# bcgsc/abyss

Measured on AMD Instinct MI355X. Metric: Mk-mers/s inserted+extended (abyss-bloom-dbg, k=64); unitig bit-exact, higher is better.
Workload: dtype u64

## Files before the change

abyss_amd/csrc/abg_core.h:

```cpp
#pragma once

#include <stdint.h>
#include <stddef.h>

#if defined(__HIPCC__)
#include <hip/hip_runtime.h>
#define ABG_HD __host__ __device__ __forceinline__
#define ABG_HDN __host__ __device__
#define ABG_HDX __host__ __device__ __attribute__((noinline))
#else
#define ABG_HD inline
#define ABG_HDN
#define ABG_HDX
#endif

namespace abg {

constexpr int MAX_NW = 6;
constexpr int MAX_HASHES = 32;
constexpr unsigned FP_TRIM = 5;

enum Dir : int { FORWARD = 0, REVERSE = 1 };
enum Sense : int { SENSE = 0, ANTISENSE = 1 };

// ... 1106 lines not shown
	uint32_t o = *counter; *counter = o + 1; return o;
}
#endif

#if defined(__HIP_DEVICE_COMPILE__)
ABG_HD void wave_count_add(uint64_t* counter, bool want)
{
	const uint64_t m = __ballot(want ? 1 : 0);
	if (m && (int)__lane_id() == __ffsll((unsigned long long)m) - 1) atomicAdd((unsigned long long*)counter, (unsigned long long)__popcll(m));
}
#else
ABG_HD void wave_count_add(uint64_t* counter, bool want) { if (want) *counter += 1; }
#endif

#if defined(__HIP_DEVICE_COMPILE__)
ABG_HD uint32_t wave_rank(bool want, uint32_t& count)
{
	const uint64_t m = __ballot(want ? 1 : 0);
	count = (uint32_t)__popcll(m);
	return (uint32_t)__popcll(m & ((1ull << __lane_id()) - 1));
}
#else
ABG_HD uint32_t wave_rank(bool want, uint32_t& count) { count = want ? 1u : 0u; return 0; }
#endif

#if defined(__HIP_DEVICE_COMPILE__)
ABG_HD uint64_t wu_cas_u64(uint64_t* p, uint64_t expect, uint64_t val, bool coop)
{
	if (!coop) return cas_u64(p, expect, val);
	uint64_t r = 0;
	if (__lane_id() == 0) r = cas_u64(p, expect, val);
	return ((uint64_t)(uint32_t)__builtin_amdgcn_readfirstlane((int)(r >> 32)) << 32) |
	       (uint32_t)__builtin_amdgcn_readfirstlane((int)(uint32_t)r);
}
ABG_HD uint32_t wu_atomic_min_u32(uint32_t* p, uint32_t v, bool coop)
{
	if (!coop) return atomic_min_u32(p, v);
	uint32_t r = 0;
	if (__lane_id() == 0) r = atomic_min_u32(p, v);
	return (uint32_t)__builtin_amdgcn_readfirstlane((int)r);
}
ABG_HD uint32_t wu_atomic_add_u32(uint32_t* p, uint32_t v, bool coop)
{
	if (!coop) return atomic_add_u32(p, v);
	uint32_t r = 0;
	if (__lane_id() == 0) r = atomic_add_u32(p, v);
// ... 1001 lines not shown
```

abyss_amd/csrc/abg_engine.h:

```cpp
#pragma once
#include "abg_walk.h"

#include <algorithm>
#include <chrono>
#include <cstdio>
#include <cstdlib>
#include <cstring>
#include <functional>
#include <future>
#include <string>
#include <type_traits>
#include <vector>

namespace abg {

struct Failure { int code; std::string msg; };
constexpr int FAIL_INVAL = -1, FAIL_NOMEM = -3, FAIL_INTERNAL = -4;
[[noreturn]] inline void fail_now(int code, const std::string& msg) { throw Failure{ code, msg }; }
inline std::string strf(const char* fmt, unsigned long long a = 0, unsigned long long b = 0)
{
	char buf[256];
	snprintf(buf, sizeof buf, fmt, a, b);
	return buf;
}
// ... 31 lines not shown
	uint32_t p2_crowded = 1u << 18;
	uint32_t p2_starved_growth = 2;
	uint32_t p2_starved = 6144;
	uint32_t slice_filter = 0;
	bool solid_plane = true;
	uint32_t classify_slots = 65536;
	uint32_t cls_both_max_mb = 1024;
	bool cls_both = true;
	bool prefetch_classify = true;
	uint32_t memo_log2 = 0;
	bool memo = true;
	uint32_t p2_max_candidates = 1u << 18;
	uint32_t t_tags = 1024;
	uint32_t commit_incremental = 1;
	uint32_t commit_dirty_max = 4096;
	uint32_t commit_dirty_log2 = 26;
	uint32_t guide_stride = 4;
	uint32_t guide_log2_max = 31;
	bool guide_seen = true;
	bool link_duplicates = true;
	bool par_commit = true;
	bool overlap_bins = true;
	bool overlap_purity = true;
	uint32_t dist_hash_all_ranks = 2;
	uint32_t dist_route_min_ranks = 4;
	uint64_t keep_insert_scratch_bytes = 16ull << 30;
	uint64_t par_commit_max_bytes = 16ull << 30;
	int verbose = 0;
};

struct Counters {
	uint64_t solid_reads = 0, visited_reads = 0, reads_processed = 0, bases_assembled = 0,
	         contig_id = 0;
};

struct BaseCodes {
	uint8_t t[256];
	BaseCodes()
	{
		for (int i = 0; i < 256; i++) t[i] = 0xFF;
		t['A'] = t['a'] = 0; t['C'] = t['c'] = 1; t['G'] = t['g'] = 2; t['T'] = t['t'] = 3;
	}
};
template <class T>
struct NoInitAlloc : std::allocator<T> {
	template <class U> struct rebind { using other = NoInitAlloc<U>; };
// ... 412 lines not shown
constexpr uint32_t TILE_PAIRS_MEAN = 1u << ABG_TILE_PAIRS_LOG2;
constexpr uint32_t TILE_SORT_MAX = 3u * TILE_PAIRS_MEAN / 2;
struct TilePair { uint32_t hlo, hhi, tj; };
constexpr uint32_t TP_T_BITS = 28, TP_T_MASK = (1u << TP_T_BITS) - 1;
ABG_HD uint64_t tp_h(const TilePair& r) { return ((uint64_t)r.hhi << 32) | r.hlo; }
ABG_HD uint32_t tp_t(const TilePair& r) { return r.tj & TP_T_MASK; }
ABG_HD uint32_t tp_j(const TilePair& r) { return r.tj >> TP_T_BITS; }
constexpr uint32_t LEAD_BIT = 0x80000000u;
struct TileEnv {
	Params p; uint8_t* cnt;
	uint64_t lo, m;
	const uint64_t* h0;
	TilePair* bins; uint32_t cap;
	uint32_t* tcur;
	uint32_t* lead;
	uint8_t* opflag;
	uint8_t* tgt;
	uint8_t* pendf;
	uint32_t* flags;
	uint32_t benign = 1;
	uint32_t lead_js = 2;
	uint32_t count_max = 0x7FFFFFFFu;
	const uint8_t* cval = nullptr;
	uint32_t* bad = nullptr;
	uint32_t bad_mask = 0;
	uint8_t* wmask = nullptr;
	uint32_t* chg = nullptr;
	uint32_t* colist = nullptr;
	uint8_t* cocnt = nullptr;
	uint32_t glog2 = 0;
};
constexpr uint32_t CO_MAX_PASSES = 15;
constexpr uint8_t PEND_NO = 0, PEND_ROUNDS = 1, PEND_CANDIDATE = 2;
constexpr uint32_t CO_LANE_SHIFT = 26, CO_MORE = 1u << 25, CO_SLOT_MASK = CO_MORE - 1, CO_DEAD = 0xFFFFFFFFu;
template <class Get, class Put>
ABG_HD void kmer_hash_run(const Params& p, Get get, uint32_t j0, uint32_t j1, Put put)
{
	if (j0 >= j1) return;
	const unsigned k = p.k;
	if (p.mask) {
		const MaskTab& m = *p.mask;
		uint64_t fh = 0, rh = 0, df = 0, dr = 0;
		for (unsigned i = 0; i < k; i++) {
			fh = srol1(fh) ^ seed_of(get(j0 + i));
			rh = srol1(rh) ^ seed_of(3u - get(j0 + k - 1 - i));
		}
// ... 257 lines not shown
		atomic_min_u64(&first[s], ((uint64_t)tp_t(r) << TILE_IDX_BITS) | i);
		atomic_add_u32(&info[s], 1);
	});
	sy.barrier();
	if (keep) {
		TilePair fst[TILE_PURITY_PER];
#pragma unroll
		for (uint32_t q = 0; q < TILE_PURITY_PER; q++) {
			const uint32_t i = tid + q * nt;
			fst[q] = bin[i < n ? (uint32_t)(first[slot[q] & 0xFFFFu] & ((1u << TILE_IDX_BITS) - 1u)) : 0u];
		}
#pragma unroll
		for (uint32_t q = 0; q < TILE_PURITY_PER; q++) {
			const uint32_t i = tid + q * nt;
			const TilePair& r = mine[q]; const TilePair& f = fst[q];
			if (i < n && (r.hlo != f.hlo || r.hhi != f.hhi || ((r.tj ^ f.tj) != 0 && tp_t(r) == tp_t(f)))) atomic_or_u32(&info[slot[q] & 0xFFFFu], 0x80000000u);
		}
	} else
	pairs([&](const TilePair& r, uint32_t, uint32_t s, uint32_t) {
		const TilePair f = bin[(uint32_t)(first[s] & ((1u << TILE_IDX_BITS) - 1u))];
		if (r.hlo != f.hlo || r.hhi != f.hhi || ((r.tj ^ f.tj) != 0 && tp_t(r) == tp_t(f))) atomic_or_u32(&info[s], 0x80000000u);
	});
	sy.barrier();
	pairs([&](const TilePair& r, uint32_t, uint32_t s, uint32_t) {
		const uint32_t inf = info[s], t = tp_t(r);
		if ((inf >> 31) || (inf & 0x7FFFFFFFu) >= e.count_max) {
			const uint32_t bit = e.p.nh <= 8 ? (1u << tp_j(r)) : 0xFFu;
			atomic_or_u32((uint32_t*)e.opflag + (t >> 2), bit << (8 * (t & 3u)));
			return;
		}
		if (tp_j(r) >= e.lead_js) return;
		const bool first_op = (uint32_t)(first[s] >> TILE_IDX_BITS) == t;
		e.lead[t] = (inf & 0x7FFFFFFFu) | (first_op ? LEAD_BIT : 0u);
	});
}
ABG_HD uint32_t bad_slot(const TileEnv& e, uint64_t pos) { return (uint32_t)(pos ^ (pos >> 27)) & e.bad_mask; }
ABG_HD void mark_bad(const TileEnv& e, uint64_t h, unsigned js)
{
	for (unsigned j = 0; j < e.p.nh && j < 8; j++)
		if ((js >> j) & 1u) { const uint32_t s = bad_slot(e, pos_i(e.p, h, j)); atomic_or_u32(&e.bad[s >> 5], 1u << (s & 31u)); }
}
ABG_HD bool any_bad(const TileEnv& e, uint64_t h, unsigned js)
{
	bool b = false;
	for (unsigned j = 0; j < e.p.nh && j < 8; j++)
		if ((js >> j) & 1u) { const uint32_t s = bad_slot(e, pos_i(e.p, h, j)); b |= ((e.bad[s >> 5] >> (s & 31u)) & 1u) != 0; }
	return b;
}
ABG_HD void op_verdict(const TileEnv& e, uint64_t t, uint8_t& tgt, uint8_t& pend, uint32_t& centry)
{
	tgt = 0; pend = PEND_ROUNDS; centry = 0;
	if (e.flags[0]) return;
	const uint32_t fl = e.opflag[t], L = e.lead[t], n = L & ~LEAD_BIT;
	if (fl && (!n || e.p.nh > 8 || !e.benign)) { if (e.bad && e.p.nh <= 8) mark_bad(e, e.h0[t], fl); return; }
	if (!fl && !(L & LEAD_BIT)) { pend = PEND_NO; return; }
	const uint64_t h = e.h0[t];
	unsigned mp = 256, ms = 256;
	unsigned cs[8];
	for (unsigned j0 = 0; j0 < e.p.nh; j0 += 4) {
		unsigned c[4];
#pragma unroll
		for (unsigned q = 0; q < 4; q++) {
			const unsigned jq = j0 + q < e.p.nh ? j0 + q : 0u;
			c[q] = e.cval ? 255u - e.cval[t * e.p.nh + jq] : e.cnt[pos_i(e.p, h, jq)];
		}
#pragma unroll
		for (unsigned q = 0; q < 4; q++) {
			const unsigned j = j0 + q;
			if (j >= e.p.nh) continue;
			if (j < 8) cs[j] = c[q];
			if ((fl >> j) & 1u) ms = c[q] < ms ? c[q] : ms; else mp = c[q] < mp ? c[q] : mp;
		}
	}
	const unsigned tg = mp + n > 255 ? 255u : mp + n;
	if (fl && ms < tg) {
		if (!e.bad) return;
// ... 125 lines not shown
	if (ld_coherent(&e.flags[0])) return;
	const uint64_t nbins = (e.m - e.lo + BIN_COUNTERS - 1) >> BIN_BITS;
	uint32_t nb[TILE_SPLIT], n = 0;
#pragma unroll
	for (uint32_t q = 0; q < TILE_SPLIT; q++) {
		const uint64_t bi = tile * TILE_SPLIT + q;
		const uint32_t f = bi < nbins ? ld_coherent(&e.tcur[bi]) : 0u;
		nb[q] = f < e.cap ? f : e.cap;
		n += nb[q];
	}
	if (!n) return;
	const uint32_t tid = sy.tid(), nt = sy.nthreads();
	const uint64_t base = e.lo + (tile << TILE_BITS);
	const uint32_t span = (uint32_t)(e.m - base < TILE_COUNTERS ? e.m - base : TILE_COUNTERS);
	uint64_t* l8 = (uint64_t*)lds;
	const uint64_t* g8 = (const uint64_t*)(e.cnt + base);
	for (uint32_t i = tid; i < span / 8; i += nt) l8[i] = g8[i];
	sy.barrier();
	bool any = false;
	constexpr uint32_t PER = TILE_SPLIT * ((TILE_SORT_MAX + 1023) / 1024);
	uint32_t mine[PER];
	uint32_t kept = 0;
	const bool keep = e.bad && nt >= 1024;
	auto raise = [&](const TilePair& r, bool first) -> bool {
		const uint8_t tg = e.tgt[tp_t(r)];
		if (!tg) return false;
		const uint32_t off = (uint32_t)(pos_i(e.p, tp_h(r), tp_j(r)) - e.lo) & (TILE_COUNTERS - 1);
		if (first && keep && kept < PER) mine[kept++] = off | ((uint32_t)tg << 16);
		if (lds[off] < tg) { lds[off] = tg; return true; }
		return false;
	};
#pragma unroll
	for (uint32_t q = 0; q < TILE_SPLIT; q++) {
		const TilePair* bin = e.bins + (tile * TILE_SPLIT + q) * e.cap;
		for (uint32_t i = tid; i < nb[q]; i += nt) any |= raise(bin[i], true);
	}
	if (e.bad) {
		for (bool again = any; sy.any(again);) {
			again = false;
			if (keep) {
#pragma unroll
				for (uint32_t q = 0; q < PER; q++)
					if (q < kept) { const uint32_t off = mine[q] & 0xFFFFu; const uint8_t tg = (uint8_t)(mine[q] >> 16); if (lds[off] < tg) { lds[off] = tg; again = true; } }
			} else {
				for (uint32_t q = 0; q < TILE_SPLIT; q++) {
					const TilePair* bin = e.bins + (tile * TILE_SPLIT + q) * e.cap;
					for (uint32_t i = tid; i < nb[q]; i += nt) again |= raise(bin[i], false);
				}
			}
		}
	}
	if (sy.any(any)) {
		uint64_t* o8 = (uint64_t*)(e.cnt + base);
		for (uint32_t i = tid; i < span / 8; i += nt) o8[i] = l8[i];
	}
}
struct SortEnv {
	TileEnv e; uint64_t T, np;
	uint64_t* key; uint32_t* val;
	uint64_t* sid;
	uint32_t* start;
	uint8_t* impure;
};
struct FSortKeys {
	SortEnv s;
	ABG_HD void operator()(uint64_t q, uint32_t) const
	{
		const uint64_t t = q / s.e.p.nh; const unsigned j = (unsigned)(q - t * s.e.p.nh);
		s.key[q] = pos_i(s.e.p, s.e.h0[t], j);
		s.val[q] = (uint32_t)t << 4 | j;
// ... 13 lines not shown
};
struct FSegImpure {
	SortEnv s;
	ABG_HD void operator()(uint64_t i, uint32_t) const
	{
		const uint64_t g = s.sid[i] - 1, f = s.start[g];
		if (i == f) return;
		const uint32_t v = s.val[i], vf = s.val[f];
		if (s.e.h0[v >> 4] != s.e.h0[vf >> 4] || (v >> 4) == (vf >> 4)) s.impure[g] = 1;
	}
};
struct FSegJudge {
	SortEnv s;
	ABG_HD void operator()(uint64_t i, uint32_t) const
	{
		const uint64_t g = s.sid[i] - 1;
		const uint32_t f = s.start[g], cnt = s.start[g + 1] - f, v = s.val[i], t = v >> 4, j = v & 15u;
		if (s.impure[g] || cnt >= s.e.count_max) {
			const uint32_t bit = s.e.p.nh <= 8 ? (1u << j) : 0xFFu;
			atomic_or_u32((uint32_t*)s.e.opflag + (t >> 2), bit << (8 * (t & 3u)));
			return;
		}
		if (j >= s.e.lead_js) return;
		s.e.lead[t] = cnt | ((s.val[f] >> 4) == t ? LEAD_BIT : 0u);
	}
};
struct FSegApply {
	SortEnv s;
	ABG_HD void operator()(uint64_t i, uint32_t) const
	{
		const uint8_t tg = s.e.tgt[s.val[i] >> 4];
		if (!tg) return;
		const uint64_t pos = s.key[i];
		uint32_t* w = (uint32_t*)(s.e.cnt + (pos & ~3ull));
		const unsigned sh = 8u * (unsigned)(pos & 3u);
		for (uint32_t old = *w;;) {
			if (((old >> sh) & 0xFFu) >= tg) return;
			const uint32_t want = (old & ~(0xFFu << sh)) | ((uint32_t)tg << sh);
			const uint32_t got = cas_u32(w, old, want);
			if (got == old) return;
			old = got;
		}
	}
};
struct FClaimList {
	Params p; const uint64_t* h0; const uint32_t* pend; uint64_t* claim; uint64_t cmask; uint32_t epoch;
// ... 1628 lines not shown
			casc_.levels = cfg_.cascade_levels;
			casc_.level_words = (m_ + 31) / 32;
			casc_.bits = (uint32_t*)be_.alloc(casc_.levels * casc_.level_words * 4);
			be_.memset(casc_.bits, 0, casc_.levels * casc_.level_words * 4);
			cnt_ = (uint8_t*)be_.alloc(8);
			vis_bytes_ = 8;
		} else {
			const uint64_t dev = be_.device_mem_bytes();
			cnt_deferred_ = cfg_.slice_filter == 1 || (cfg_.slice_filter == 0 && dev && (double)m_ * 1.3 > (double)dev * 0.9);
			if (!cnt_deferred_) {
				cnt_ = (uint8_t*)be_.alloc(m_ + 64 * (MAX_RANKS + 1));
				be_.memset(cnt_, 0, m_);
			}
			vis_bytes_ = (m_ / 8 + 4 + 3) & ~3ull;
		}
		vis_ = (uint8_t*)be_.alloc(vis_bytes_);
		be_.memset(vis_, 0, vis_bytes_);
		cstate_ = (CommitState*)be_.alloc(sizeof(CommitState));
		be_.memset(cstate_, 0, sizeof(CommitState));
		scal_ = (uint64_t*)be_.alloc(64);
	}
	~Engine()
	{
		free_counters(); be_.free(vis_); if (both_) be_.free(both_); be_.free(cstate_); be_.free(scal_);
		free_archive();
		if (casc_.bits) be_.free(casc_.bits);
		if (mask_d_) be_.free(mask_d_);
		if (T_) be_.free(T_);
		if (Tk_) { be_.free(Tk_); be_.free(Tv_); }
		if (pcA_) be_.free(pcA_);
		if (la_pool_c_) be_.free(la_pool_c_);
		if (la_pool_c2_) be_.free(la_pool_c2_);
		if (guide_tab_) be_.free(guide_tab_);
		if (guide_seen_) be_.free(guide_seen_);
		if (gtab_.hmin) free_tab(gtab_);
		free_shared();
		free_insert();
		free_walk();
		if (cend_.hmin) free_tab(cend_);
		if (memo_tab_.hmin) free_tab(memo_tab_);
		if (plane_) be_.free(plane_);
		if (wstats_) be_.free(wstats_);
	}
	void reset()
	{
		if (casc_.bits) be_.memset(casc_.bits, 0, casc_.levels * casc_.level_words * 4);
// ... 248 lines not shown
	}
	void load_packed(const Batch& b, const uint64_t* koff_h) { load_packed(b, cut_ranges_host(koff_h, b.n)); }
	void load_packed(const Batch& b) { load_packed(b, cut_ranges(b.koff, b.n)); }
	void load_packed(const Batch& b, const std::vector<OpRange>& ranges)
	{
		need_counters();
		cnt_loaded_ = true;
		{
			uint32_t len0 = 0;
			if (b.n) be_.d2h(&len0, b.len, 4);
			const uint32_t nk0 = len0 >= p_.k ? len0 - p_.k + 1 : 0;
			const uint32_t parts = (nk0 + 31) / 32;
			hash_run_ = parts ? std::min<uint32_t>(32, std::max<uint32_t>(8, (nk0 + parts - 1) / parts)) : 8;
		}
		ensure_insert();
		memo_valid_ = false; plane_valid_ = false;
		last_rounds_ = 0;
		const bool pipe = tiled_ && bins_alt_ != nullptr && !routed();
		for (size_t i = 0; i < ranges.size(); i++) {
			if (!pipe) { insert_range(b, ranges[i], false); continue; }
			if (i == 0) stage_bins(b, ranges[0]);
			be_.wait_side_scope();
			std::swap(h0_, h0_alt_); std::swap(bins_, bins_alt_); std::swap(tcur_, tcur_alt_); stage_flag_ ^= 1u;
			if (lead_alt_) { std::swap(lead_, lead_alt_); std::swap(opflag_, opflag_alt_); }
			const bool staged = staged_ok_;
			purity_done_ = staged && staged_purity_;
			const uint32_t cur_flag = stage_flag_ ^ 1u;
			stage_next_ = nullptr;
			if (i + 1 < ranges.size()) stage_next_ = [this, &b, &ranges, i]() { stage_bins(b, ranges[i + 1]); };
			insert_range(b, ranges[i], staged, 2 + cur_flag);
			if (stage_next_) { stage_next_(); stage_next_ = nullptr; }
		}
	}
	void stage_bins(const Batch& b, const OpRange& rg)
	{
		const uint64_t s = rg.s, e = rg.e;
		const uint64_t T = rg.k1 - rg.k0;
		staged_ok_ = false;
		if (T == 0 || T > batch_ops_ || T >= 0xFFFFFFFFull) return;
		Batch v = b;
		v.woff = b.woff + s; v.len = b.len + s; v.n = e - s; v.koff = b.koff + s;
		const uint64_t kbase = rg.k0;
		uint32_t* flag = pend_n_ + 2 + stage_flag_;
		uint64_t* h0 = h0_alt_;
		const bool part = dist();
		TileEnv te{ p_, cnt_, part ? own_lo_ : 0, part ? own_lo_ + own_span_ : m_, h0_alt_, bins_alt_, tile_cap_, tcur_alt_, lead_alt_ ? lead_alt_ : lead_,
			opflag_alt_ ? opflag_alt_ : opflag_, tgt_, pendf_, flag, cfg_.benign_sharers ? 1u : 0u, part ? 16u : 2u, part ? 254u : 0x7FFFFFFFu };
		const uint64_t R = part ? (uint64_t)comm_.world : 1, me = part ? (uint64_t)comm_.rank : 0;
		if (part && R > cfg_.dist_hash_all_ranks) {
			const uint64_t chunk = ((T + R - 1) / R + 7) & ~7ull;
			std::vector<uint64_t> c(R, chunk * 8), d(R);
			for (uint64_t q = 0; q < R; q++) d[q] = q * chunk * 8;
			const uint64_t a = std::min(T, me * chunk), bnd = std::min(T, a + chunk);
			if (bnd > a) {
				be_.side_scope_begin("hash_staged");
				dispatch_nw([&](auto nw) { FHashOps<(decltype(nw)::value & 7)> f{ p_, v, h0, bnd, kbase, a, hash_run_ }; be_.launch((bnd - a + hash_run_ - 1) / hash_run_, f, "hash_ops"); });
				be_.side_scope_end();
				be_.wait_side_scope();
			}
			c_all_gather_v(h0, c.data(), d.data());
		}
		be_.side_scope_begin("hash_bin_staged");
		be_.memset(tcur_alt_, 0, ntiles_ * 4);
		be_.memset(flag, 0, 4);
		be_.memset(ccur_, 0, ncoarse_ * 4);
		if (!part || R <= cfg_.dist_hash_all_ranks)
			dispatch_nw([&](auto nw) { FHashOps<(decltype(nw)::value & 7)> f{ p_, v, h0, T, kbase, 0, hash_run_ }; be_.launch((T + hash_run_ - 1) / hash_run_, f, "hash_ops"); });
		BinEnv bn{ te, T, coarse_, coarse_cap_, ccur_, cshift_, ncoarse_ };
		FBinCoarse f1{ bn };
		be_.launch_tiles((T + BIN_CHUNK_OPS - 1) / BIN_CHUNK_OPS, f1, "bin_coarse");
		const uint32_t cpb = (coarse_cap_ + BIN_CHUNK_PAIRS - 1) / BIN_CHUNK_PAIRS;
		FBinFine f2{ bn, cpb };
		be_.launch_tiles((uint64_t)ncoarse_ * cpb, f2, "bin_fine");
		staged_purity_ = false;
		if (lead_alt_) {
			be_.memset(lead_alt_, 0, T * 4);
			be_.memset(opflag_alt_, 0, (T + 3) & ~3ull);
			FTilePurity fp{ te };
			be_.launch_tiles(ntiles_, fp, "tile_purity");
			staged_purity_ = true;
		}
		be_.side_scope_end();
		staged_ok_ = true;
	}
	bool staged_ok_ = false; uint32_t stage_flag_ = 0;
	bool purity_done_ = false;
	std::function<void()> stage_next_;

	void assemble_packed(const Batch& b, uint8_t* results_host,
	    const std::function<void(const ContigOut&)>& sink)
	{
		const bool timing = getenv("ABG_HOST_TIMING") != nullptr;
		const auto tnow = []() { return std::chrono::duration<double>(std::chrono::steady_clock::now().time_since_epoch()).count(); };
		const double t_in = tnow();
		const auto mark = [&](const char* what) { if (timing) { be_.sync(); fprintf(stderr, "[host] assemble_packed +%.3f s: %s\n", tnow() - t_in, what); } };
		need_counters();
		gather_counters();
		if (insert_scratch_bytes_ > cfg_.keep_insert_scratch_bytes) free_insert();
		mark("counters final, PASS 1's scratch given back where it is large");
		ensure_walk();
		mark("walkers' pools and tables");
		ensure_plane();
		ensure_both();
		mark("bit plane, two-bit array");
		ensure_archive(b);
		mark("archive");
		build_guide(b);
		mark("guide");
// ... 124 lines not shown
		});
		guide_.tab = guide_tab_;
		guide_slots_ = guide_.mask + 1;
		if (cfg_.guide_seen) {
			const uint64_t need = nwords * 16, total = be_.device_mem_bytes();
			if (guide_seen_ && guide_seen_bytes_ < need) { be_.free(guide_seen_); guide_seen_ = nullptr; }
			if (!guide_seen_ && (!total || need <= total / 24)) { guide_seen_ = (uint8_t*)be_.try_alloc(need); guide_seen_bytes_ = need; }
			if (guide_seen_) { be_.memset(guide_seen_, 0, need); guide_.seen = guide_seen_; }
		}
	}
	uint64_t next_batch_size() const
	{
		if (last_candidates_ > cfg_.p2_crowded) return std::max<uint64_t>(p2_batch_ / 2, 1024);
		if (last_candidates_ < cfg_.p2_starved) return std::min<uint64_t>(p2_batch_ * cfg_.p2_starved_growth, 8 * cfg_.p2_max_batch);
		return std::min<uint64_t>(p2_batch_ * cfg_.p2_growth, cfg_.p2_max_batch);
	}
	void clear_wstats()
	{
		be_.memset(wstats_, 0, WSTAT_N * 8);
	}
	struct Stats { uint64_t rounds = 0, walked = 0, rewalked = 0, candidates = 0, breaks = 0, insert_rounds = 0, commit_rounds = 0, generated = 0;
	               uint64_t bulk_calls = 0, bulk_steps = 0, lin_steps = 0, guide_slots = 0, chain_steps = 0, batch_cuts = 0, overflows = 0, memo_hits = 0, memo_adds = 0;
	               uint64_t tiled_ops = 0, tiled_pending = 0, tile_overflows = 0, cls_covered_reads = 0, archive_bases = 0, cls_decided_reads = 0;
	               uint64_t commit_rounds_incremental = 0, commit_dirty_records = 0, commit_first_chunk_decided = 0; };
	Stats stats()
	{
		Stats s = stats_;
		if (wstats_) {
			uint64_t v[WSTAT_N];
			be_.d2h(v, wstats_, sizeof v);
			s.bulk_calls = v[WSTAT_BULK_CALLS]; s.bulk_steps = v[WSTAT_BULK_STEPS]; s.lin_steps = v[WSTAT_LIN_STEPS]; s.chain_steps = v[WSTAT_CHAIN_STEPS];
			s.memo_hits = v[WSTAT_MEMO_HITS]; s.memo_adds = v[WSTAT_MEMO_ADDS];
			s.cls_covered_reads = v[WSTAT_CLS_COVERED]; s.cls_decided_reads = v[WSTAT_CLS_DECIDED];
		}
		if (arc_.seq && arc_valid_) { uint64_t u = 0; be_.d2h(&u, arc_.used, 8); s.archive_bases = std::min(u, arc_.cap) - ARC_HEAD; }
		s.guide_slots = guide_slots_;
		return s;
	}

  private:
	BE& be_;
	Config cfg_;
	Params p_;
	uint64_t m_ = 0, vis_bytes_ = 0;
	uint8_t* cnt_ = nullptr;
	uint8_t* vis_ = nullptr;
// ... 92 lines not shown
		std::vector<uint64_t> c(comm_.world), d(comm_.world);
		for (int q = 0; q < comm_.world; q++) { d[q] = (uint64_t)q * own_chunk_; c[q] = own_chunk_; }
		c_all_gather_v(cnt_, c.data(), d.data());
		cnt_partial_ = false;
	}
	Counters counters_;
	Stats stats_;
	uint64_t last_rounds_ = 0;
	uint64_t p2_batch_ = 0;
	uint64_t* h0_ = nullptr; uint64_t* claim_[2] = { nullptr, nullptr };
	uint32_t* pend_[2] = { nullptr, nullptr }; uint32_t* pend_n_ = nullptr; uint32_t epoch_ = 1;
	uint64_t batch_ops_ = 0;
	uint32_t hash_run_ = 8;
	uint64_t insert_scratch_bytes_ = 0;
	uint32_t claim_log2_ = 0;
	bool tiled_ = false; uint64_t ntiles_ = 0, napply_ = 0; uint32_t tile_cap_ = 0;
	TilePair* coarse_ = nullptr; uint32_t* ccur_ = nullptr; uint32_t coarse_cap_ = 0, cshift_ = 0, ncoarse_ = 0;
	TilePair* bins_ = nullptr; uint32_t* tcur_ = nullptr; uint32_t* lead_ = nullptr; uint8_t* opflag_ = nullptr; uint8_t* tgt_ = nullptr; uint8_t* pendf_ = nullptr;
	uint64_t* h0_alt_ = nullptr; TilePair* bins_alt_ = nullptr; uint32_t* tcur_alt_ = nullptr;
	uint32_t* colist_ = nullptr; uint8_t* cocnt_ = nullptr;
	uint64_t* pgrp_ = nullptr;
	uint8_t* wmask_ = nullptr; uint32_t* bad_ = nullptr; uint32_t* cochg_ = nullptr;
	uint32_t* lead_alt_ = nullptr; uint8_t* opflag_alt_ = nullptr;
	bool staged_purity_ = false;
	Guide guide_{ nullptr, 0, nullptr, 0, nullptr }; uint64_t* guide_tab_ = nullptr; uint32_t guide_log2_ = 0;
	uint8_t* guide_seen_ = nullptr; uint64_t guide_seen_bytes_ = 0;
	BulkScratch* bulk_pool_ = nullptr; uint64_t* wstats_ = nullptr; uint64_t guide_slots_ = 0;
	SuccMemo memo_{ nullptr, nullptr, nullptr, 0 }; WalkTab memo_tab_{ nullptr, nullptr, nullptr, 0 }; bool memo_valid_ = false; uint64_t memo_gen_ = 0;
	bool walk_ready_ = false;
	WalkTab wtab_{}, cend_{ nullptr, nullptr, nullptr, 0 };
	uint32_t wtab_log2_ = 0;
	uint64_t wtab_per_walker_ = 1536;
	void* tb_pool_ = nullptr; VKey* tbk_pool_ = nullptr; VKey* la_pool_ = nullptr; uint8_t* lbuf_ = nullptr; uint8_t* rbuf_ = nullptr;
	uint8_t* pool_ = nullptr; uint64_t pool_cap_ = 0; uint64_t* pool_used_ = nullptr;
	ContigRec* recs_ = nullptr; uint32_t rec_cap_ = 0; uint32_t* rec_used_ = nullptr;
	uint32_t* order_ = nullptr; uint32_t* order_n_ = nullptr;
	uint32_t walk_tb_cap_ = 0, walk_buf_cap_ = 0, wslots_ = 0, cslots_ = 0;
	uint64_t* kh_ = nullptr; uint64_t* rkh_ = nullptr; uint64_t* dbg_ = nullptr;
	uint64_t cend_count_ = 0;
	uint8_t* read_flag_ = nullptr;
	uint64_t last_candidates_ = 0;
	VKey* la_pool_c_ = nullptr;
	VKey* la_pool_c2_ = nullptr;
	uint64_t pre_first_ = 0, pre_n_ = 0;
	std::function<void()> prefetch_;

// ... 89 lines not shown
		uint64_t nb = batch_ops_;
		if (tiled_) {
			cshift_ = 0;
			while ((ntiles_ >> cshift_) > 512 && cshift_ < 12) cshift_++;
			ncoarse_ = (uint32_t)((ntiles_ + (1ull << cshift_) - 1) >> cshift_);
			{
				const uint64_t mean = (nb * p_.nh + ncoarse_ * R - 1) / (ncoarse_ * R);
				uint64_t sq = 1;
				while (sq * sq < mean) sq++;
				coarse_cap_ = (uint32_t)(mean + 8 * sq + 256);
			}
			coarse_ = (TilePair*)be_.alloc((uint64_t)ncoarse_ * coarse_cap_ * sizeof(TilePair));
			ccur_ = (uint32_t*)be_.alloc(ncoarse_ * 4 + 64);
			bins_ = (TilePair*)be_.alloc(ntiles_ * tile_cap_ * sizeof(TilePair));
			tcur_ = (uint32_t*)be_.alloc(ntiles_ * 4 + 64);
			if (cfg_.overlap_bins) {
				bins_alt_ = (TilePair*)be_.try_alloc(ntiles_ * tile_cap_ * sizeof(TilePair));
				if (bins_alt_) {
					tcur_alt_ = (uint32_t*)be_.alloc(ntiles_ * 4 + 64);
					h0_alt_ = (uint64_t*)be_.alloc((nb + 8 * R + 8) * 8);
					if (cfg_.overlap_purity && !routed()) {
						lead_alt_ = (uint32_t*)be_.alloc(nb * 4);
						opflag_alt_ = (uint8_t*)be_.alloc(nb + 8);
					}
				}
			}
			lead_ = (uint32_t*)be_.alloc(nb * 4);
			opflag_ = (uint8_t*)be_.alloc(nb + 8);
			tgt_ = (uint8_t*)be_.alloc(nb);
			pendf_ = (uint8_t*)be_.alloc(nb + 8);
			pgrp_ = (uint64_t*)be_.alloc((nb / PEND_GROUP + 2) * 8);
			if (!routed() && cfg_.cosettle && cfg_.benign_sharers && p_.nh <= 8) {
				wmask_ = (uint8_t*)be_.alloc(nb);
				bad_ = (uint32_t*)be_.alloc((1ull << cfg_.cosettle_log2) / 8);
				cochg_ = (uint32_t*)be_.alloc((CO_MAX_PASSES + 1) * 4);
				colist_ = (uint32_t*)be_.alloc((nb + 64) * 4);
				cocnt_ = (uint8_t*)be_.alloc((nb >> BE::ITEM_GROUP_LOG2) + 64);
			}
			if (dist()) tred_ = (uint8_t*)be_.alloc((bad_ ? 3 + p_.nh : 2) * nb + 256);
			if (routed()) {
				rown_ = (((nb + R - 1) / R + 7) & ~7ull);
				const uint64_t mean = rown_ * p_.nh / R;
				uint64_t sq = 1;
				while (sq * sq < mean) sq++;
				rcap_ = (uint32_t)(mean + 8 * sq + 1024);
				if (const char* e = getenv("ABG_ROUTE_CAP")) rcap_ = (uint32_t)std::max(1, atoi(e));
				rsend_ = (TilePair*)be_.alloc((uint64_t)R * rcap_ * sizeof(TilePair));
				rrecv_cap_ = (uint64_t)R * rcap_;
				rrecv_ = (TilePair*)be_.alloc(rrecv_cap_ * sizeof(TilePair));
				rslot_ = (uint32_t*)be_.alloc(rown_ * p_.nh * 4);
				rcur_ = (uint32_t*)be_.alloc((MAX_RANKS + 2) * 4);
// ... 5 lines not shown
		h0_ = (uint64_t*)be_.alloc((nb + 8 * R + 8) * 8);
		{
			const uint64_t pairs = nb * p_.nh / (tiled_ ? 4 : 1);
			uint32_t log2 = 16;
			while (log2 < cfg_.claim_log2 && (1ull << log2) < 8 * pairs) log2++;
			for (;; log2--) {
				claim_[0] = (uint64_t*)be_.try_alloc(8ull << log2);
				claim_[1] = claim_[0] ? (uint64_t*)be_.try_alloc(8ull << log2) : nullptr;
				if (claim_[1] || log2 <= 16) break;
				if (claim_[0]) be_.free(claim_[0]);
			}
			if (!claim_[1]) fail_now(FAIL_NOMEM, "no device memory for the insert claim tables");
			claim_log2_ = log2;
		}
		for (int i = 0; i < 2; i++) {
			be_.memset(claim_[i], 0xFF, 8ull << claim_log2_);
			pend_[i] = (uint32_t*)be_.alloc(nb * 4);
		}
		pend_n_ = (uint32_t*)be_.alloc(16);
		be_.memset(pend_n_, 0, 16);
		if (dist()) dres_ = (uint8_t*)be_.alloc(std::max<uint64_t>(nb, (uint64_t)cfg_.drain_threshold * 32));
		dlost_ = (uint8_t*)be_.alloc(nb);
		insert_scratch_bytes_ = nb * (8 + 4 + 4 + 1) + (16ull << claim_log2_);
		if (tiled_) insert_scratch_bytes_ += ((uint64_t)ncoarse_ * coarse_cap_ + ntiles_ * tile_cap_ * (bins_alt_ ? 2 : 1)) * sizeof(TilePair) + nb * (bins_alt_ ? 15 : 7);
	}
	void free_insert()
	{
		if (!h0_) return;
		if (tiled_) { be_.free(coarse_); be_.free(ccur_); be_.free(bins_); be_.free(tcur_); be_.free(lead_); be_.free(opflag_); be_.free(tgt_); be_.free(pendf_); be_.free(pgrp_); pgrp_ = nullptr; tiled_ = false; }
		if (bad_) { be_.free(wmask_); be_.free(bad_); be_.free(cochg_); be_.free(colist_); be_.free(cocnt_); wmask_ = nullptr; bad_ = nullptr; cochg_ = nullptr; colist_ = nullptr; cocnt_ = nullptr; }
		if (tred_) { be_.free(tred_); tred_ = nullptr; }
		if (rsend_) {
			be_.free(rsend_); be_.free(rrecv_); be_.free(rslot_); be_.free(rcur_); be_.free(rrep_out_); be_.free(rrep_in_); be_.free(rtgt_out_); be_.free(rtgt_in_); be_.free(rpendf_);
			rsend_ = nullptr;
		}
		if (bins_alt_) { be_.free(bins_alt_); be_.free(tcur_alt_); be_.free(h0_alt_); bins_alt_ = nullptr; tcur_alt_ = nullptr; h0_alt_ = nullptr; }
		if (lead_alt_) { be_.free(lead_alt_); be_.free(opflag_alt_); lead_alt_ = nullptr; opflag_alt_ = nullptr; }
		if (dres_) { be_.free(dres_); dres_ = nullptr; }
		be_.free(dlost_);
		be_.free(h0_);
		for (int i = 0; i < 2; i++) { be_.free(claim_[i]); be_.free(pend_[i]); }
		be_.free(pend_n_);
		h0_ = nullptr;
		insert_scratch_bytes_ = 0;
	}
	void insert_range(const Batch& b, const OpRange& rg, bool staged, uint32_t flag_word = 1)
	{
		const uint64_t s = rg.s, e = rg.e;
		uint64_t T = rg.k1 - rg.k0;
		if (T == 0) return;
		loaded_ops_ += T;
		if (T > batch_ops_ || T >= 0xFFFFFFFFull) {
			fail_now(FAIL_INTERNAL, strf("a single sequence has more k-mers (%llu) than insert_batch_kmers", T));
		}
		Batch v = b;
		v.woff = b.woff + s; v.len = b.len + s; v.n = e - s;
		v.koff = b.koff + s;
		const uint64_t kbase = rg.k0;
		uint64_t cmask = (1ull << claim_log2_) - 1;
		if (epoch_ > 0xFFFFFF00u) {
			for (int i = 0; i < 2; i++) be_.memset(claim_[i], 0xFF, 8ull << claim_log2_);
			epoch_ = 1;
		}
		uint64_t* ccur = claim_[0];
		uint64_t* cnext = claim_[1];
		if (dist()) {
			if (tiled_ && routed()) insert_tiles_routed(v, T, cmask, kbase);
			else if (tiled_) insert_tiles_dist(v, T, cmask, kbase, staged, staged ? flag_word : 1);
			else {
				FHashClaimT<true> fc{ p_, v, h0_, T, ccur, cmask, epoch_, own_lo_, own_span_, kbase };
				be_.launch((T + HC_RUN - 1) / HC_RUN, fc, "hash_claim");
				insert_rounds_dist(T, cmask, nullptr, T);
			}
			return;
		}
		uint64_t npend = T;
		const uint32_t* pin = nullptr;
		uint32_t* pout = pend_[0];
		bool claimed = false;
		if (tiled_) {
			if (!staged) flag_word = 1;
			TileEnv te{ p_, cnt_, 0, m_, h0_, bins_, tile_cap_, tcur_, lead_, opflag_, tgt_, pendf_, pend_n_ + flag_word, cfg_.benign_sharers ? 1u : 0u };
			const bool judged = staged && purity_done_;
			if (!judged) {
				be_.memset(lead_, 0, T * 4);
				be_.memset(opflag_, 0, (T + 3) & ~3ull);
			}
			be_.memset(pend_n_, 0, 8);
			if (!staged) {
				be_.memset(tcur_, 0, ntiles_ * 4);
				dispatch_nw([&](auto nw) { FHashOps<(decltype(nw)::value & 7)> f{ p_, v, h0_, T, kbase, 0, hash_run_ }; be_.launch((T + hash_run_ - 1) / hash_run_, f, "hash_ops"); });
				BinEnv bn{ te, T, coarse_, coarse_cap_, ccur_, cshift_, ncoarse_ };
				be_.memset(ccur_, 0, ncoarse_ * 4);
				FBinCoarse f1{ bn };
				be_.launch_tiles((T + BIN_CHUNK_OPS - 1) / BIN_CHUNK_OPS, f1, "bin_coarse");
				const uint32_t cpb = (coarse_cap_ + BIN_CHUNK_PAIRS - 1) / BIN_CHUNK_PAIRS;
				FBinFine f2{ bn, cpb };
				be_.launch_tiles((uint64_t)ncoarse_ * cpb, f2, "bin_fine");
			}
			SortBufs sb;
			bool sorted = false;
			if (cfg_.sorted_overflow) {
				uint32_t over = 0;
				be_.d2h(&over, pend_n_ + flag_word, 4);
				if (over) {
// ... 1141 lines not shown
```

abyss_amd/csrc/abg_host.h:

```cpp
#pragma once
#include "abg_engine.h"
#include "../../include/abyss_amd.h"

#include <cctype>
#include <cmath>
#include <map>
#include <string>
#include <atomic>
#include <chrono>
#include <future>
#include <memory>
#include <thread>

namespace abg {
static_assert(FAIL_NOMEM == ABG_ENOMEM && FAIL_INTERNAL == ABG_EINTERNAL, "Failure codes are the C ABI's");


struct FContainsSolid {
	Params p; const uint64_t* h0; const uint8_t* cnt; uint8_t* out;
	ABG_HD void operator()(uint64_t t, uint32_t) const { out[t] = solid_contains(p, cnt, h0[t]) ? 1 : 0; }
};
struct FExpand {
	Params p; const uint64_t* h0; uint64_t* out;
	ABG_HD void operator()(uint64_t t, uint32_t) const
// ... 58 lines not shown
		if (const char* e = getenv("ABG_P2_FIRST_BATCH")) cfg.p2_first_batch = strtoull(e, 0, 10);
		if (const char* e = getenv("ABG_P2_MAX_BATCH")) cfg.p2_max_batch = strtoull(e, 0, 10);
		if (const char* e = getenv("ABG_PAR_COMMIT")) cfg.par_commit = atoi(e) != 0;
		if (const char* e = getenv("ABG_T_TAGS")) cfg.t_tags = (uint32_t)std::max(2, atoi(e));
		if (const char* e = getenv("ABG_COMMIT_INCREMENTAL")) cfg.commit_incremental = (uint32_t)std::min(2, std::max(0, atoi(e)));
		if (const char* e = getenv("ABG_COMMIT_DIRTY_MAX")) cfg.commit_dirty_max = (uint32_t)std::max(0, atoi(e));
		if (const char* e = getenv("ABG_COMMIT_DIRTY_LOG2")) cfg.commit_dirty_log2 = (uint32_t)std::min(34, std::max(10, atoi(e)));
		if (const char* e = getenv("ABG_PAR_COMMIT_MAX_GB")) cfg.par_commit_max_bytes = strtoull(e, 0, 10) << 30;
		if (const char* e = getenv("ABG_COMPACT_THRESHOLD")) cfg.compact_threshold = strtoull(e, 0, 10);
		if (const char* e = getenv("ABG_TILED")) cfg.tiled_insert = atoi(e) != 0;
		if (const char* e = getenv("ABG_DIST_ROUTE_MIN")) cfg.dist_route_min_ranks = (uint32_t)atoi(e);
		if (const char* e = getenv("ABG_BENIGN")) cfg.benign_sharers = atoi(e) != 0;
		if (const char* e = getenv("ABG_CLS_ARCHIVE")) cfg.cls_archive = atoi(e) != 0;
		if (const char* e = getenv("ABG_CLS_DEBUG_SKIP")) cfg.cls_debug_skip = (uint32_t)atoi(e);
		if (const char* e = getenv("ABG_CLS_ARCHIVE_MAX_MB")) cfg.cls_archive_max_mb = (uint32_t)std::max(0, atoi(e));
		if (const char* e = getenv("ABG_SORTED_OVERFLOW")) cfg.sorted_overflow = atoi(e) != 0;
		if (const char* e = getenv("ABG_COSETTLE")) cfg.cosettle = atoi(e) != 0;
		if (const char* e = getenv("ABG_CLS_BOTH")) cfg.cls_both = atoi(e) != 0;
		if (const char* e = getenv("ABG_CLS_BOTH_MAX_MB")) cfg.cls_both_max_mb = (uint32_t)std::max(0, atoi(e));
		if (const char* e = getenv("ABG_COSETTLE_PASSES")) cfg.cosettle_passes = (uint32_t)std::max(1, atoi(e));
		if (const char* e = getenv("ABG_COSETTLE_LOG2")) cfg.cosettle_log2 = (uint32_t)std::min(25, std::max(5, atoi(e)));
		if (const char* e = getenv("ABG_LINK_DUPS")) cfg.link_duplicates = atoi(e) != 0;
		if (const char* e = getenv("ABG_OVERLAP_PURITY")) cfg.overlap_purity = atoi(e) != 0;
		if (const char* e = getenv("ABG_OVERLAP_BINS")) cfg.overlap_bins = atoi(e) != 0;
		if (const char* e = getenv("ABG_PREFETCH")) cfg.prefetch_classify = atoi(e) != 0;
		if (const char* e = getenv("ABG_ASYNC_LOAD")) cfg.async_load = atoi(e) != 0;
		if (const char* e = getenv("ABG_CLS_SLOTS")) cfg.classify_slots = (uint32_t)std::max(64, atoi(e));
		if (const char* e = getenv("ABG_SOLID_PLANE")) cfg.solid_plane = atoi(e) != 0;
		if (const char* e = getenv("ABG_MEMO")) cfg.memo = atoi(e) != 0;
		if (const char* e = getenv("ABG_P2_MAX_CANDIDATES")) cfg.p2_max_candidates = (uint32_t)std::max(1, atoi(e));
		if (const char* e = getenv("ABG_P2_STARVED_GROWTH")) cfg.p2_starved_growth = (uint32_t)std::max(2, atoi(e));
		if (const char* e = getenv("ABG_P2_STARVED")) cfg.p2_starved = (uint32_t)atoi(e);
		if (const char* e = getenv("ABG_P2_GROWTH")) cfg.p2_growth = (uint32_t)std::max(2, atoi(e));
		if (const char* e = getenv("ABG_DRAIN_THRESHOLD")) cfg.drain_threshold = (uint32_t)strtoul(e, 0, 10);
		if (const char* e = getenv("ABG_GUIDE_STRIDE")) cfg.guide_stride = (uint32_t)strtoul(e, 0, 10);
		if (const char* e = getenv("ABG_GUIDE_SEEN")) cfg.guide_seen = atoi(e) != 0;
		if (const char* e = getenv("ABG_GUIDE_LOG2_MAX")) cfg.guide_log2_max = (uint32_t)std::min(36, std::max(10, atoi(e)));
		if (!be.ok()) return fail(ABG_ENODEV, be.why());
		eng = new Engine<BE>(be, cfg);
		return ABG_OK;
	}

	int load_seqs(const char* seqs, const uint64_t* off, uint64_t n) { return load_seqs_v(1, &seqs, &off, &n); }
	int load_seqs_v(uint32_t nchunks, const char* const* seqs_v, const uint64_t* const* off_v, const uint64_t* n_v)
	{
		const uint32_t k = cfg.k;
// ... 744 lines not shown
```

Measured before the change: 1638.

## Skip lead stores for singleton counts and mask apply-phase target lookups

```diff
diff --git a/abyss_amd/csrc/abg_core.h b/abyss_amd/csrc/abg_core.h
--- a/abyss_amd/csrc/abg_core.h
+++ b/abyss_amd/csrc/abg_core.h
@@ -1152,6 +1152,20 @@
 }
 #else
 ABG_HD uint32_t wave_rank(bool want, uint32_t& count) { count = want ? 1u : 0u; return 0; }
+#endif
+
+#if defined(__HIP_DEVICE_COMPILE__)
+ABG_HD void wave_put_bit(uint64_t* words, uint32_t i, bool v)
+{
+	const uint64_t m = __ballot(v ? 1 : 0);
+	if (!(i & 63u)) words[i >> 6] = m;
+}
+#else
+ABG_HD void wave_put_bit(uint64_t* words, uint32_t i, bool v)
+{
+	if (!(i & 63u)) words[i >> 6] = 0;
+	words[i >> 6] |= (uint64_t)(v ? 1u : 0u) << (i & 63u);
+}
 #endif
 
 #if defined(__HIP_DEVICE_COMPILE__)
diff --git a/abyss_amd/csrc/abg_engine.h b/abyss_amd/csrc/abg_engine.h
--- a/abyss_amd/csrc/abg_engine.h
+++ b/abyss_amd/csrc/abg_engine.h
@@ -77,6 +77,8 @@
 	bool par_commit = true;
 	bool overlap_bins = true;
 	bool overlap_purity = true;
+	bool apply_mask = true;
+	bool lead_implicit = true;
 	uint32_t dist_hash_all_ranks = 2;
 	uint32_t dist_route_min_ranks = 4;
 	uint64_t keep_insert_scratch_bytes = 16ull << 30;
@@ -535,6 +537,9 @@
 	uint32_t lead_js = 2;
 	uint32_t count_max = 0x7FFFFFFFu;
 	const uint8_t* cval = nullptr;
+	uint32_t lead_implicit = 0;
+	uint64_t* amask = nullptr;
+	uint64_t* lead_stat = nullptr;
 	uint32_t* bad = nullptr;
 	uint32_t bad_mask = 0;
 	uint8_t* wmask = nullptr;
@@ -838,16 +843,25 @@
 		if (r.hlo != f.hlo || r.hhi != f.hhi || ((r.tj ^ f.tj) != 0 && tp_t(r) == tp_t(f))) atomic_or_u32(&info[s], 0x80000000u);
 	});
 	sy.barrier();
-	pairs([&](const TilePair& r, uint32_t, uint32_t s, uint32_t) {
+	uint64_t* amask = e.amask ? e.amask + tile * ((e.cap + 63u) >> 6) : nullptr;
+	pairs([&](const TilePair& r, uint32_t i, uint32_t s, uint32_t) {
 		const uint32_t inf = info[s], t = tp_t(r);
+		bool may_lead = true;
 		if ((inf >> 31) || (inf & 0x7FFFFFFFu) >= e.count_max) {
 			const uint32_t bit = e.p.nh <= 8 ? (1u << tp_j(r)) : 0xFFu;
 			atomic_or_u32((uint32_t*)e.opflag + (t >> 2), bit << (8 * (t & 3u)));
-			return;
-		}
-		if (tp_j(r) >= e.lead_js) return;
-		const bool first_op = (uint32_t)(first[s] >> TILE_IDX_BITS) == t;
-		e.lead[t] = (inf & 0x7FFFFFFFu) | (first_op ? LEAD_BIT : 0u);
+		} else {
+			const bool first_op = (uint32_t)(first[s] >> TILE_IDX_BITS) == t;
+			may_lead = first_op;
+			if (tp_j(r) < e.lead_js) {
+				if (e.lead_implicit && inf == 1u) { if (e.lead_stat) e.lead_stat[1]++; }
+				else {
+					if (e.lead_stat) e.lead_stat[0]++;
+					e.lead[t] = (inf & 0x7FFFFFFFu) | (first_op ? LEAD_BIT : 0u);
+				}
+			}
+		}
+		if (amask) wave_put_bit(amask, i, may_lead);
 	});
 }
 ABG_HD uint32_t bad_slot(const TileEnv& e, uint64_t pos) { return (uint32_t)(pos ^ (pos >> 27)) & e.bad_mask; }
@@ -863,11 +877,18 @@
 		if ((js >> j) & 1u) { const uint32_t s = bad_slot(e, pos_i(e.p, h, j)); b |= ((e.bad[s >> 5] >> (s & 31u)) & 1u) != 0; }
 	return b;
 }
+ABG_HD uint32_t lead_of(const TileEnv& e, uint64_t t, uint32_t fl)
+{
+	const uint32_t L = e.lead[t];
+	if (L || !e.lead_implicit) return L;
+	const uint32_t mask = (1u << (e.lead_js < e.p.nh ? e.lead_js : e.p.nh)) - 1u;
+	return (fl & mask) != mask ? (1u | LEAD_BIT) : 0u;
+}
 ABG_HD void op_verdict(const TileEnv& e, uint64_t t, uint8_t& tgt, uint8_t& pend, uint32_t& centry)
 {
 	tgt = 0; pend = PEND_ROUNDS; centry = 0;
 	if (e.flags[0]) return;
-	const uint32_t fl = e.opflag[t], L = e.lead[t], n = L & ~LEAD_BIT;
+	const uint32_t fl = e.opflag[t], L = lead_of(e, t, fl), n = L & ~LEAD_BIT;
 	if (fl && (!n || e.p.nh > 8 || !e.benign)) { if (e.bad && e.p.nh <= 8) mark_bad(e, e.h0[t], fl); return; }
 	if (!fl && !(L & LEAD_BIT)) { pend = PEND_NO; return; }
 	const uint64_t h = e.h0[t];
@@ -1039,8 +1060,9 @@
 	uint32_t mine[PER];
 	uint32_t kept = 0;
 	const bool keep = e.bad && nt >= 1024;
-	auto raise = [&](const TilePair& r, bool first) -> bool {
-		const uint8_t tg = e.tgt[tp_t(r)];
+	auto raise = [&](const TilePair& r, bool may_lead, bool first) -> bool {
+		const uint8_t g = e.tgt[may_lead ? tp_t(r) : 0u];
+		const uint8_t tg = may_lead ? g : (uint8_t)0;
 		if (!tg) return false;
 		const uint32_t off = (uint32_t)(pos_i(e.p, tp_h(r), tp_j(r)) - e.lo) & (TILE_COUNTERS - 1);
 		if (first && keep && kept < PER) mine[kept++] = off | ((uint32_t)tg << 16);
@@ -1050,7 +1072,11 @@
 #pragma unroll
 	for (uint32_t q = 0; q < TILE_SPLIT; q++) {
 		const TilePair* bin = e.bins + (tile * TILE_SPLIT + q) * e.cap;
-		for (uint32_t i = tid; i < nb[q]; i += nt) any |= raise(bin[i], true);
+		if (e.amask) {
+			const uint64_t* am = e.amask + (tile * TILE_SPLIT + q) * ((e.cap + 63u) >> 6);
+			for (uint32_t i = tid; i < nb[q]; i += nt) { const TilePair r = bin[i]; const uint64_t w = am[i >> 6]; any |= raise(r, ((w >> (i & 63u)) & 1u) != 0, true); }
+		} else
+		for (uint32_t i = tid; i < nb[q]; i += nt) any |= raise(bin[i], true, true);
 	}
 	if (e.bad) {
 		for (bool again = any; sy.any(again);) {
@@ -1062,7 +1088,7 @@
 			} else {
 				for (uint32_t q = 0; q < TILE_SPLIT; q++) {
 					const TilePair* bin = e.bins + (tile * TILE_SPLIT + q) * e.cap;
-					for (uint32_t i = tid; i < nb[q]; i += nt) again |= raise(bin[i], false);
+					for (uint32_t i = tid; i < nb[q]; i += nt) again |= raise(bin[i], true, false);
 				}
 			}
 		}
@@ -1122,6 +1148,8 @@
 			return;
 		}
 		if (j >= s.e.lead_js) return;
+		if (s.e.lead_implicit && cnt == 1u) { if (s.e.lead_stat) s.e.lead_stat[1]++; return; }
+		if (s.e.lead_stat) s.e.lead_stat[0]++;
 		s.e.lead[t] = cnt | ((s.val[f] >> 4) == t ? LEAD_BIT : 0u);
 	}
 };
@@ -2796,6 +2824,8 @@
 	}
 	~Engine()
 	{
+		if (BE::ITEM_GROUP_LOG2 == 0 && getenv("ABG_LEAD_COUNT"))
+			fprintf(stderr, "lead_stores made=%llu skipped=%llu\n", (unsigned long long)stats_.lead_stores[0], (unsigned long long)stats_.lead_stores[1]);
 		free_counters(); be_.free(vis_); if (both_) be_.free(both_); be_.free(cstate_); be_.free(scal_);
 		free_archive();
 		if (casc_.bits) be_.free(casc_.bits);
@@ -3090,7 +3120,7 @@
 			if (i == 0) stage_bins(b, ranges[0]);
 			be_.wait_side_scope();
 			std::swap(h0_, h0_alt_); std::swap(bins_, bins_alt_); std::swap(tcur_, tcur_alt_); stage_flag_ ^= 1u;
-			if (lead_alt_) { std::swap(lead_, lead_alt_); std::swap(opflag_, opflag_alt_); }
+			if (lead_alt_) { std::swap(lead_, lead_alt_); std::swap(opflag_, opflag_alt_); std::swap(amask_, amask_alt_); }
 			const bool staged = staged_ok_;
 			purity_done_ = staged && staged_purity_;
 			const uint32_t cur_flag = stage_flag_ ^ 1u;
@@ -3114,6 +3144,7 @@
 		const bool part = dist();
 		TileEnv te{ p_, cnt_, part ? own_lo_ : 0, part ? own_lo_ + own_span_ : m_, h0_alt_, bins_alt_, tile_cap_, tcur_alt_, lead_alt_ ? lead_alt_ : lead_,
 			opflag_alt_ ? opflag_alt_ : opflag_, tgt_, pendf_, flag, cfg_.benign_sharers ? 1u : 0u, part ? 16u : 2u, part ? 254u : 0x7FFFFFFFu };
+		if (!part) { te.lead_implicit = cfg_.lead_implicit ? 1u : 0u; te.lead_stat = lead_stat(); te.amask = amask_alt_; }
 		const uint64_t R = part ? (uint64_t)comm_.world : 1, me = part ? (uint64_t)comm_.rank : 0;
 		if (part && R > cfg_.dist_hash_all_ranks) {
 			const uint64_t chunk = ((T + R - 1) / R + 7) & ~7ull;
@@ -3152,6 +3183,7 @@
 		staged_ok_ = true;
 	}
 	bool staged_ok_ = false; uint32_t stage_flag_ = 0;
+	uint64_t* lead_stat() { return BE::ITEM_GROUP_LOG2 == 0 ? stats_.lead_stores : nullptr; }
 	bool purity_done_ = false;
 	std::function<void()> stage_next_;
 
@@ -3322,6 +3354,7 @@
 	struct Stats { uint64_t rounds = 0, walked = 0, rewalked = 0, candidates = 0, breaks = 0, insert_rounds = 0, commit_rounds = 0, generated = 0;
 	               uint64_t bulk_calls = 0, bulk_steps = 0, lin_steps = 0, guide_slots = 0, chain_steps = 0, batch_cuts = 0, overflows = 0, memo_hits = 0, memo_adds = 0;
 	               uint64_t tiled_ops = 0, tiled_pending = 0, tile_overflows = 0, cls_covered_reads = 0, archive_bases = 0, cls_decided_reads = 0;
+	               uint64_t lead_stores[2] = { 0, 0 };
 	               uint64_t commit_rounds_incremental = 0, commit_dirty_records = 0, commit_first_chunk_decided = 0; };
 	Stats stats()
 	{
@@ -3460,6 +3493,7 @@
 	uint64_t* pgrp_ = nullptr;
 	uint8_t* wmask_ = nullptr; uint32_t* bad_ = nullptr; uint32_t* cochg_ = nullptr;
 	uint32_t* lead_alt_ = nullptr; uint8_t* opflag_alt_ = nullptr;
+	uint64_t* amask_ = nullptr; uint64_t* amask_alt_ = nullptr;
 	bool staged_purity_ = false;
 	Guide guide_{ nullptr, 0, nullptr, 0, nullptr }; uint64_t* guide_tab_ = nullptr; uint32_t guide_log2_ = 0;
 	uint8_t* guide_seen_ = nullptr; uint64_t guide_seen_bytes_ = 0;
@@ -3595,11 +3629,13 @@
 					if (cfg_.overlap_purity && !routed()) {
 						lead_alt_ = (uint32_t*)be_.alloc(nb * 4);
 						opflag_alt_ = (uint8_t*)be_.alloc(nb + 8);
+						if (cfg_.apply_mask && !dist()) amask_alt_ = (uint64_t*)be_.alloc(ntiles_ * ((tile_cap_ + 63u) >> 6) * 8);
 					}
 				}
 			}
 			lead_ = (uint32_t*)be_.alloc(nb * 4);
 			opflag_ = (uint8_t*)be_.alloc(nb + 8);
+			if (cfg_.apply_mask && !dist()) amask_ = (uint64_t*)be_.alloc(ntiles_ * ((tile_cap_ + 63u) >> 6) * 8);
 			tgt_ = (uint8_t*)be_.alloc(nb);
 			pendf_ = (uint8_t*)be_.alloc(nb + 8);
 			pgrp_ = (uint64_t*)be_.alloc((nb / PEND_GROUP + 2) * 8);
@@ -3651,7 +3687,8 @@
 		if (dist()) dres_ = (uint8_t*)be_.alloc(std::max<uint64_t>(nb, (uint64_t)cfg_.drain_threshold * 32));
 		dlost_ = (uint8_t*)be_.alloc(nb);
 		insert_scratch_bytes_ = nb * (8 + 4 + 4 + 1) + (16ull << claim_log2_);
-		if (tiled_) insert_scratch_bytes_ += ((uint64_t)ncoarse_ * coarse_cap_ + ntiles_ * tile_cap_ * (bins_alt_ ? 2 : 1)) * sizeof(TilePair) + nb * (bins_alt_ ? 15 : 7);
+		if (tiled_) insert_scratch_bytes_ += ((uint64_t)ncoarse_ * coarse_cap_ + ntiles_ * tile_cap_ * (bins_alt_ ? 2 : 1)) * sizeof(TilePair) + nb * (bins_alt_ ? 15 : 7)
+			+ ntiles_ * ((tile_cap_ + 63u) >> 6) * 8 * ((amask_ ? 1 : 0) + (amask_alt_ ? 1 : 0));
 	}
 	void free_insert()
 	{
@@ -3665,6 +3702,8 @@
 		}
 		if (bins_alt_) { be_.free(bins_alt_); be_.free(tcur_alt_); be_.free(h0_alt_); bins_alt_ = nullptr; tcur_alt_ = nullptr; h0_alt_ = nullptr; }
 		if (lead_alt_) { be_.free(lead_alt_); be_.free(opflag_alt_); lead_alt_ = nullptr; opflag_alt_ = nullptr; }
+		if (amask_) { be_.free(amask_); amask_ = nullptr; }
+		if (amask_alt_) { be_.free(amask_alt_); amask_alt_ = nullptr; }
 		if (dres_) { be_.free(dres_); dres_ = nullptr; }
 		be_.free(dlost_);
 		be_.free(h0_);
@@ -3710,6 +3749,7 @@
 		if (tiled_) {
 			if (!staged) flag_word = 1;
 			TileEnv te{ p_, cnt_, 0, m_, h0_, bins_, tile_cap_, tcur_, lead_, opflag_, tgt_, pendf_, pend_n_ + flag_word, cfg_.benign_sharers ? 1u : 0u };
+			te.lead_implicit = cfg_.lead_implicit ? 1u : 0u; te.lead_stat = lead_stat(); te.amask = amask_;
 			const bool judged = staged && purity_done_;
 			if (!judged) {
 				be_.memset(lead_, 0, T * 4);
diff --git a/abyss_amd/csrc/abg_host.h b/abyss_amd/csrc/abg_host.h
--- a/abyss_amd/csrc/abg_host.h
+++ b/abyss_amd/csrc/abg_host.h
@@ -104,6 +104,8 @@
 		if (const char* e = getenv("ABG_COSETTLE_LOG2")) cfg.cosettle_log2 = (uint32_t)std::min(25, std::max(5, atoi(e)));
 		if (const char* e = getenv("ABG_LINK_DUPS")) cfg.link_duplicates = atoi(e) != 0;
 		if (const char* e = getenv("ABG_OVERLAP_PURITY")) cfg.overlap_purity = atoi(e) != 0;
+		if (const char* e = getenv("ABG_LEAD_IMPLICIT")) cfg.lead_implicit = atoi(e) != 0;
+		if (const char* e = getenv("ABG_APPLY_MASK")) cfg.apply_mask = atoi(e) != 0;
 		if (const char* e = getenv("ABG_OVERLAP_BINS")) cfg.overlap_bins = atoi(e) != 0;
 		if (const char* e = getenv("ABG_PREFETCH")) cfg.prefetch_classify = atoi(e) != 0;
 		if (const char* e = getenv("ABG_ASYNC_LOAD")) cfg.async_load = atoi(e) != 0;
```

Result: faster. 1709, median of 6 (+4.3%).
